# Thomi6York/pbrt-v2-skin

Measured on AMD Instinct MI355X. Metric: Msamples/s (skin.pbrt C2 pixel loop) + Mo()-gather roofline, higher is better.
Workload: dtype f32; 1 GPU; C2: skin.pbrt 1024x1024 64 spp (1024x1024, 64 spp per GPU), 128x128 tiles; scene=skin.pbrt, sampler=hash, triangles=15864, irradiance_points=2216917, tiles=64, skin_tiles=8, mo_common_grid=True

## Files before the change

### include/mpss.h

```cpp
#ifndef MPSS_H
#define MPSS_H
#include <stdint.h>

#ifdef __cplusplus
extern "C" {
#endif

#define MPSS_NBANDS 30

enum {
    MPSS_OK = 0,
    MPSS_ERR_INVALID = -1,
    MPSS_ERR_INTERNAL = -2,
    MPSS_ERR_HIP = -3,
    MPSS_ERR_NOMEM = -4
};

typedef struct mpss_ctx mpss_ctx;

typedef struct {
    int device;
    int max_depth;
    float max_error;
    float min_sample_distance;
// ... 50 lines not shown
int mpss_add_layeredskin(mpss_ctx *ctx, const mpss_layeredskin *m, uint32_t *material_id);
int mpss_update_layeredskin(mpss_ctx *ctx, uint32_t material_id, const mpss_layeredskin *m);
int mpss_build_counts(mpss_ctx *ctx, uint64_t counts[4]);
int mpss_set_material_tables(mpss_ctx *ctx, const float *rd_table, uint32_t length, const float *rcp,
                             const float *rho_hd, uint32_t n_rho, const float *albedo, int is_monte_carlo,
                             uint32_t *material_id);
int mpss_add_dipole_material(mpss_ctx *ctx, const float *sigma_a, const float *sigmap_s, float eta,
                             uint32_t *material_id);
int mpss_get_material_tables(mpss_ctx *ctx, uint32_t material_id, float *rd_table, uint32_t *length, float *rcp,
                             float *rho_hd, uint32_t *n_rho, float *total_reflectance);
int mpss_get_gather_info(mpss_ctx *ctx, uint32_t id, int *common_grid, float *rel_err, float *l1_err);

typedef struct {
    int width, height;
    const float *texels;
    int is_float;
    float shift, scale, gamma;
    int wrap;
    int trilinear;
    float max_anisotropy;
    float uscale, vscale, udelta, vdelta;
} mpss_imagemap;
void mpss_imagemap_defaults(mpss_imagemap *t);
int mpss_add_imagemap(mpss_ctx *ctx, const mpss_imagemap *t, uint32_t *texture_id);
int mpss_set_material_textures(mpss_ctx *ctx, uint32_t material_id, int32_t albedo_texture, int32_t bump_texture);

int mpss_set_irradiance_points(mpss_ctx *ctx, uint32_t n, const float *p, const float *nrm, const float *E,
                               const float *area);
int mpss_octree_info(mpss_ctx *ctx, uint32_t *n_nodes, uint32_t *max_depth, uint32_t *n_points);
int mpss_octree_export(mpss_ctx *ctx, void *nodes, float *node_et, float *pt_hdr, float *pt_e, int32_t *pt_index);

int mpss_mo_batch(mpss_ctx *ctx, uint32_t material_id, uint32_t q, const float *p_dev, float *mo_dev,
                  int32_t *counters_dev, void *stream);

int mpss_add_mesh(mpss_ctx *ctx, uint32_t nverts, const float *P, const float *N, const float *S, const float *uv,
                  uint32_t ntris, const int32_t *indices, const float *obj_to_world, const float *world_to_obj,
                  int reverse_orientation, uint32_t material_id);
int mpss_add_sphere_light(mpss_ctx *ctx, const float *center, float radius, const float *Lemit, int nsamples);
int mpss_add_infinite_light(mpss_ctx *ctx, const float *L, int nsamples, const float *light_to_world,
                            const float *world_to_light);
int mpss_add_infinite_light_map(mpss_ctx *ctx, const float *L, int nsamples, const float *light_to_world,
                                const float *world_to_light, int width, int height, const float *texels);
int mpss_set_camera(mpss_ctx *ctx, const float *raster_to_camera, const float *camera_to_world, int xres, int yres);
int mpss_set_surface_points(mpss_ctx *ctx, uint32_t n, const void *records);
int mpss_get_surface_points(mpss_ctx *ctx, void *records, uint32_t *n);
int mpss_load_pointsfile(mpss_ctx *ctx, const char *path);
int mpss_save_pointsfile(mpss_ctx *ctx, const char *path);
int mpss_get_irradiance(mpss_ctx *ctx, float *E, uint32_t *n);
int mpss_replay_samples(mpss_ctx *ctx, int spp, float *out, uint64_t *n_floats, int *k);
int mpss_preprocess(mpss_ctx *ctx, uint32_t seed);
int mpss_render_tile(mpss_ctx *ctx, int spp, uint32_t seed, int x0, int x1, int y0, int y1, float *xyzw_dev,
                     void *stream);
int mpss_render_tiles(mpss_ctx *ctx, int spp, uint32_t seed, int n, const int32_t *rects, float *const *xyzw_dev,
                      void *stream);

int mpss_tile_costs(mpss_ctx *ctx, int n, const int32_t *rects, int64_t *sss_hits, int64_t *surf_hits);

typedef struct {
    double ms_irradiance, ms_camera, ms_shade, ms_film;
    int64_t n_irradiance, n_camera, n_shade, n_film;
    int64_t samples;
    int64_t sss_samples;
    int64_t mo_nodes;
    int64_t mo_points;
    int64_t group_nodes[8], group_points[8];
    int32_t group_bands[8][4];
// ... 96 lines not shown
```

### pbrt-v2-skin_amd/csrc/context.cpp

```cpp
#include "context.h"
#include "spectral.h"

#include <cstring>

namespace mpss {

Context::Context(const mpss_config &cfg) : cfg_(cfg) {
    int ndev = 0;
    MPSS_HIP(hipGetDeviceCount(&ndev));
    if (cfg.device < 0 || cfg.device >= ndev)
        throw Error(MPSS_ERR_INVALID, "mpss_create: device ordinal " + std::to_string(cfg.device) +
                                          " out of range (" + std::to_string(ndev) + " HIP devices)");
    if (cfg.mo_near_field != 10236 && cfg.mo_near_field != 5088)
        throw Error(MPSS_ERR_INVALID, "mpss_create: mo_near_field must be 10236 or 5088");
    if (cfg.mo_common_grid != 0 && cfg.mo_common_grid != 1)
        throw Error(MPSS_ERR_INVALID, "mpss_create: mo_common_grid must be 0 or 1");
    if (cfg.mo_band_dealing != 0 && cfg.mo_band_dealing != 1)
        throw Error(MPSS_ERR_INVALID, "mpss_create: mo_band_dealing must be 0 or 1");
    max_error_ = cfg.max_error;
    min_dist_ = cfg.min_sample_distance;
    if (cfg.quick_render) {
        max_error_ *= 4.f;
        min_dist_ *= 4.f;
    }
// ... 45 lines not shown
    try {
        std::lock_guard<std::mutex> g(mu_);
        ws_free_.emplace_back(ws);
        if (ws_free_.size() > kMaxIdleWorkspaces) {
            drop = std::move(ws_free_.front());
            ws_free_.erase(ws_free_.begin());
        }
    } catch (...) {
        if (!drop) drop.reset(ws);
    }
    drop.reset();
    return e;
}

void Context::release_ws(RenderWorkspace *ws, hipStream_t stream) { MPSS_HIP(release_ws_nothrow(ws, stream)); }

void Context::quiesce_locked() {
    idle_.wait(mu_, [&] { return inflight_ == 0; });
    MPSS_HIP(hipDeviceSynchronize());
}

void Context::end_inflight() {
    std::lock_guard<std::mutex> g(mu_);
    if (--inflight_ == 0) idle_.notify_all();
}

void Context::ensure_layouts() {
    if (!have_octree_) return;
    for (const auto &m : materials_)
        if (!m->dipole) dev_octree_.ensure_layout(m->dev_profile.groups);
}

void Context::mo_batch(uint32_t mid, int q, const float *p_dev, float *out_dev, int32_t *counters_dev,
                       hipStream_t stream) {
    activate();
    RenderWorkspace *ws = nullptr;
    const BandLayout *layout = nullptr;
    const Material *m = nullptr;
    int mode;
    GatherOpts opts;
    {
        std::lock_guard<std::mutex> g(mu_);
        opts = gather_opts();
        if (!have_octree_) throw Error(MPSS_ERR_INVALID, "no irradiance points: call mpss_set_irradiance_points first");
        if (mid >= materials_.size()) throw Error(MPSS_ERR_INVALID, "unknown material id " + std::to_string(mid));
        m = materials_[mid].get();
        if (m->no_bssrdf)
            throw Error(MPSS_ERR_INVALID, "material " + std::to_string(mid) + " has no profile (genprofile false)");
        mode = cfg_.exact_mo;
        if (m->dipole) {
            mode = -1;
        } else if (m->rgb && mode != 0) {
            mode = -2;
        } else if (mode == 0) {
            layout = &dev_octree_.ensure_layout(m->dev_profile.groups);
            ws = acquire_ws();
        }
        ++inflight_;
    }
    InflightGuard guard{this, ws, stream};
    if (mode == -1) {
        launch_mo_dipole(dev_octree_, m->dev_dipole.ptr, max_error_, q, p_dev, out_dev, NB, counters_dev, stream);
        return;
    }
    if (mode == -2) {
        launch_mo_rgb(dev_octree_, m->dev_rgb.ptr, m->dev_rgb_rcp.ptr, m->rgb_rcp, m->profile.length, max_error_, q,
                      p_dev, nullptr, nullptr, nullptr, 0, out_dev, NB, counters_dev, stream);
        return;
    }
    int *perm = nullptr;
    if (ws) {
        ws->reserve(ws->perm, (size_t)(((int64_t)q + 1023) / 1024 * 1024));
        perm = ws->perm.ptr;
        if (ws->pending) MPSS_HIP(hipStreamWaitEvent(stream, ws->done, 0));
    }
    launch_mo_gather(dev_octree_, layout, m->dev_profile, max_error_, q, p_dev, out_dev, NB, counters_dev,
                     ws ? ws->work.ptr : nullptr, perm, mode, opts, stream);
    guard.release();
}

void Context::activate() const { MPSS_HIP(hipSetDevice(cfg_.device)); }

void Context::gather_info(uint32_t id, int *common_grid, float *rel_err, float *l1_err) const {
    std::lock_guard<std::mutex> g(mu_);
    if (id >= materials_.size()) throw Error(MPSS_ERR_INVALID, "unknown material id " + std::to_string(id));
    const Material &m = *materials_[id];
    const bool band = !m.dipole;
    const int lay = cfg_.mo_near_field == 10236 ? 0 : 1;
    const bool on = band && cfg_.exact_mo == 0 && cfg_.mo_common_grid != 0 &&
                    (lay == 0 ? m.dev_profile.cg.on : m.dev_profile.cg_half.on);
    *common_grid = on ? 1 : 0;
    for (int c = 0; c < NB; ++c) {
        if (rel_err) rel_err[c] = band ? m.dev_profile.cg_rel_err[lay][c] : 0.f;
        if (l1_err) l1_err[c] = band ? m.dev_profile.cg_l1_err[lay][c] : 0.f;
    }
}

void Context::material_tables(uint32_t id, float *rd, uint32_t *len, float *rcp, float *rho, uint32_t *n_rho,
                              float *total) const {
    std::lock_guard<std::mutex> g(mu_);
    if (id >= materials_.size()) throw Error(MPSS_ERR_INVALID, "unknown material id " + std::to_string(id));
    const Material &m = *materials_[id];
    *len = (uint32_t)m.profile.length;
    *n_rho = (uint32_t)m.rho.hd.size();
    if (rd) memcpy(rd, m.profile.table.data(), sizeof(float) * m.profile.table.size());
    if (rcp) memcpy(rcp, m.profile.rcp, sizeof(float) * NB);
    if (rho) memcpy(rho, m.rho.hd.data(), sizeof(float) * m.rho.hd.size());
    if (total) memcpy(total, m.profile.total_reflectance, sizeof(float) * NB);
}

void Context::common_grid(uint32_t id, int near_field, float *rows, uint32_t *n_rows, int32_t *bands, float *rg,
// ... 344 lines not shown
```

### pbrt-v2-skin_amd/csrc/context.h

```cpp
#pragma once
#include <condition_variable>
#include <memory>
#include <mutex>
#include <vector>

#include "../../include/mpss.h"
#include "common.h"
#include "dipole.h"
#include "material.h"
#include "mo_kernel.h"
#include "octree.h"
#include "pixel_filter.h"
#include "replay.h"
#include "scene.h"
#include "texture_build.h"
#include "tile_plan.h"

namespace mpss {

struct RenderScene;

struct Material {
    ProfileTables profile;
    RhoTable rho;
// ... 69 lines not shown
                     float *u0lim, float *u1lim, float *u1start, uint32_t *row0, uint32_t *ubase, float *rel_err,
                     float *l1_err, float *ua, float *hinv, int *ok) const;
    void build_counts(uint64_t counts[4]) const;
    void set_irradiance_points(int n, const float *p, const float *nrm, const float *E, const float *area);
    const DeviceOctree &octree() const;
    void export_octree(void *nodes, float *node_et, float *pt_hdr, float *pt_e, int32_t *pt_index);
    uint32_t add_imagemap(const mpss_imagemap &m);
    void set_material_textures(uint32_t material, int albedo, int bump);
    std::vector<const TexView *> host_bump_views() const;
    float max_error() const { return max_error_; }
    GatherOpts gather_opts() const {
        GatherOpts o;
        o.near_field = cfg_.mo_near_field;
        o.steal = cfg_.mo_work_stealing != 0;
        o.count_noprune = cfg_.count_traversal == 2;
        o.common_grid = cfg_.mo_common_grid != 0;
        return o;
    }
    const mpss_config &config() const { return cfg_; }

    void add_mesh(uint32_t nv, const float *P, const float *N, const float *S, const float *uv, uint32_t nt,
                  const int32_t *idx, const float *o2w, const float *w2o, bool reverse, uint32_t material);
    void add_sphere_light(const float *c, float r, const float *Lemit, int nsamples);
    void add_infinite_light(const float *L, int nsamples, const float *l2w, const float *w2l, int W = 0, int H = 0,
                            const float *texels = nullptr);
    void set_camera(const float *r2c, const float *c2w, int xres, int yres);
    void set_surface_points(uint32_t n, const SurfacePoint *pts);
    void preprocess(uint32_t seed);
    void tessellate_on_gpu();
    void find_poisson_points(uint32_t seed);
    void render_tiles(int spp, uint32_t seed, int n, const int32_t *rects, float *const *outs, hipStream_t stream);
    void replay_samples(int spp, float *out, uint64_t *n_floats, int *k);
    void check_replay_lds(int spp, const char *who) const;
    void mo_batch(uint32_t mid, int q, const float *p_dev, float *out_dev, int32_t *counters_dev, hipStream_t stream);
    void tile_costs(int n, const int32_t *rects, int64_t *sss, int64_t *surf);
    std::vector<SurfacePoint> surface_points() const {
        std::lock_guard<std::mutex> g(mu_);
        return points_;
    }
    std::vector<float> irradiance() const {
        std::lock_guard<std::mutex> g(mu_);
        return irradiance_;
    }
    std::unique_lock<std::mutex> lock_device() const {
        activate();
        return std::unique_lock<std::mutex>(mu_);
    }
    bool has_octree() const { return have_octree_; }
    mpss_render_stats render_stats();
    void reset_render_stats();
    void set_grid_builder(bool on_host) {
        std::lock_guard<std::mutex> g(mu_);
        grid_on_host_ = on_host;
    }
    void set_pixel_filter(const PixelFilter &f) {
        std::lock_guard<std::mutex> g(mu_);
        filter_ = f;
    }
    void set_instrumentation(bool timing, int counting) {
        std::lock_guard<std::mutex> g(mu_);
        cfg_.kernel_timing = timing;
        cfg_.count_traversal = counting;
    }

private:
    void activate() const;
    void upload_scene();
// ... 117 lines not shown
```

### pbrt-v2-skin_amd/csrc/mo_band.h

```cpp
#pragma once
#include <cmath>
#include <cstdlib>

#include "common.h"
#include "common_grid_types.h"
#include "octree.h"

namespace mpss {

constexpr int kHist = 13;


struct RgbK {
    float w[4];
    float x[3][4];
    float y[3][4];
};

struct BandTree {
    const NodeHdr *__restrict__ nodes;
    const float4 *__restrict__ band_et;
    const float4 *__restrict__ pt_hdr;
    const float4 *__restrict__ band_e;
    const float4 *__restrict__ band_ew;
    const float *__restrict__ table;
    BandGroups groups;
    float grcp[kGroups][4];
    float grcp_max[kGroups];
    const float *leaf_r2;
    int L, n_nodes, n_points;
    float max_error, prune_f;
    CommonGrid cg;
    CommonGrid cg_half;
    int lband[kGroups][4];
    const float *rgb_refl;
    RgbK rgb_k[kGroups];
};

struct PruneLimit {
    float rcp_min, prune_f;
};
inline PruneLimit prune_limit(int L, float rcp_min) {
    const float r = rcp_min > 0.f ? rcp_min : 0.f;
// ... 290 lines not shown
                                          int hist[kHist]) {
    CgRec r;
    const float u = d2 * c.rg;
    const uint64_t m_lds = __builtin_amdgcn_ballot_w64(u < c.u0lim);
    const uint64_t m_in = __builtin_amdgcn_ballot_w64(u < c.u1lim);
    const bool p_lds = __builtin_amdgcn_inverse_ballot_w64(m_lds);
    const bool p_row = __builtin_amdgcn_inverse_ballot_w64(m_in & ~m_lds);
    const bool p_own = __builtin_amdgcn_inverse_ballot_w64(~(m_in | m_lds));
    const int path = p_lds ? 1 : (p_row ? 0 : 2);
    const float v = __builtin_fminf(u, __builtin_fmaf(u, c.hinv, c.hc));
    uint32_t orow = 32u * ((uint32_t)v + c.rowoff);
    asm volatile("" : "+v"(orow));
    if (p_lds) cg_lds(b, c, d2, r);
    asm volatile("" : "+v"(r.p01), "+v"(r.p23)::"memory");
    if (p_own) cg_own<COUNT>(b, c, table, d2, r, hist);
    asm volatile("" ::: "memory");
    if (p_row) {
        gf4v *row = (gf4v *)((const __attribute__((address_space(1))) char *)c.tab + orow);
        r.p01 = row[0];
        r.p23 = row[1];
        if (COUNT) cg_count_rows<COUNT>((uint64_t)(uintptr_t)c.tab + orow, hist);
        const float t = __builtin_amdgcn_fractf(v);
#pragma unroll
        for (int j = 0; j < 4; ++j) r.f[j] = t;
    }
    cg_count<COUNT>(b, c, d2, path, hist);
    return r;
}

template <bool COUNT>
__device__ __forceinline__ void cg_fix(const BandLane &b, const CgLane &c, const float *table, float d2, CgRec &r,
                                       int hist[kHist]) {
    const bool bad = r.p01.x != r.p01.x;
    if (__builtin_amdgcn_ballot_w64(bad) != 0 && bad) cg_own<COUNT>(b, c, table, d2, r, hist);
}
template <bool COUNT>
__device__ __forceinline__ void cg_fix2(const BandLane &b, const CgLane &c, const float *table, float d2a,
                                        CgRec &ra, float d2b, CgRec &rb, int hist[kHist]) {
    const bool bad_a = ra.p01.x != ra.p01.x, bad_b = rb.p01.x != rb.p01.x;
    if (__builtin_amdgcn_ballot_w64(bad_a || bad_b) != 0) {
        if (bad_a) cg_own<COUNT>(b, c, table, d2a, ra, hist);
        if (bad_b) cg_own<COUNT>(b, c, table, d2b, rb, hist);
    }
}

__device__ __forceinline__ CgRec cg_fetch_near(const BandLane &b, const CgLane &c, float d2) {
    CgRec r;
    cg_lds(b, c, d2, r);
    return r;
}

template <bool RGB = false>
__device__ __forceinline__ void cg_combine(const CgRec &r, const float e[4], f2v acc[2], lds_float *rk = nullptr) {
    float rd[4];
    const RdPair v[4] = {{r.p01.x, r.p01.y}, {r.p01.z, r.p01.w}, {r.p23.x, r.p23.y}, {r.p23.z, r.p23.w}};
#pragma unroll
    for (int j = 0; j < 4; ++j) {
        const float t = r.f[j];
        float d;
        asm("v_sub_f32 %0, %1, %2" : "=v"(d) : "v"(v[j].b), "v"(v[j].a));
        asm("v_fma_f32 %0, %1, %2, %3" : "=v"(rd[j]) : "v"(t), "v"(d), "v"(v[j].a));
    }
    float o[4];
    if (RGB) from_rgb4_fused(rk, rd[0], rd[1], rd[2], o);
    const float *x = RGB ? o : rd;
#pragma unroll
    for (int h = 0; h < 2; ++h)
        acc[h] = __builtin_elementwise_fma(f2v{x[2 * h], x[2 * h + 1]}, f2v{e[2 * h], e[2 * h + 1]}, acc[h]);
}

template <bool POINT, bool COUNT, int KLDS, bool RGB = false>
__device__ __forceinline__ void band_rd_accumulate(const BandLane &b, float d2, const float e[4], float w, f2v acc[2],
                                                   int hist[kHist], lds_float *rk = nullptr) {
    float f[4];
    RdPair v[4];
    band_rd_fetch<COUNT, KLDS>(b, d2, f, v, hist);
    band_rd_combine<POINT, RGB>(f, v, e, w, acc, rk);
}

__device__ __forceinline__ bool dw_below(float a, float d, float m, float m_lo, float m_hi) {
    const uint64_t m_below = __builtin_amdgcn_ballot_w64(a < d * m_lo);
    const uint64_t m_above = __builtin_amdgcn_ballot_w64(a > d * m_hi);
    bool below = __builtin_amdgcn_inverse_ballot_w64(m_below);
    if (__builtin_amdgcn_inverse_ballot_w64(~(m_below | m_above))) below = (a / d) < m;
    return below;
}

template <bool COUNT, int KLDS, bool VROWS, bool CG = false, bool RGB = false>
__device__ __forceinline__ void mo_band_traverse(const BandTree &a, int grp, float px, float py, float pz, bool valid,
                                                 float out[4], int &k_nodes, int &k_pts, int &w_nodes, int &w_pts,
                                                 int hist[kHist], const float *lt) {
    BandLane b;
#pragma unroll
    for (int j = 0; j < 4; ++j) {
        const int c = a.lband[grp][j];
        b.rcp[j] = a.grcp[grp][j];
        b.off[j] = (uint32_t)(c >= 0 ? c : 0) * (uint32_t)a.L;
    }
    lds_float *rk = (lds_float *)lt + 4 * near_row<KLDS>() - 28;
    b.lm1 = (uint32_t)(a.L - 1);
    const uint32_t lm2 = b.lm1 - 1u;
    b.klim = (uint32_t)KLDS < lm2 ? (uint32_t)KLDS : lm2;
    b.gspan = b.lm1 - b.klim;
#pragma unroll
    for (int j = 0; j < 4; ++j) b.tb[j] = VROWS ? in_vgprs(a.table + b.off[j]) : a.table + b.off[j];
    b.lt = lt;
    b.ltl = (lds_float *)lt;
    CgLane cl;
    if (CG) {
        cl.tab = a.cg.tab;
        cl.rowoff = a.cg.row0[grp] - a.cg.ubase[grp];
        cl.rg = a.cg.rg[grp];
        cl.u0lim = a.cg.u0lim[grp];
        cl.u1lim = a.cg.u1lim[grp];
        cl.hinv = in_vgpr(a.cg.hinv[grp]);
        cl.hc = a.cg.hc[grp];
#pragma unroll
        for (int j = 0; j < 4; ++j) {
            cl.lrow[j] = a.cg.lrow[grp][j];
            cl.off[j] = b.off[j];
        }
        cl.lm1 = (uint32_t)a.L - 1u;
        cl.zoff = 4u * (uint32_t)NB * (uint32_t)a.L;
    }
    f2v acc[2] = {f2v{0.f, 0.f}, f2v{0.f, 0.f}};
    const float lds_r2_lim = !a.leaf_r2 ? 0.f : CG ? a.cg.lds_r2[grp] : (float)b.klim / (a.grcp_max[grp] * 1.00001f);
    const uint32_t lds_code = __float_as_uint(lds_r2_lim) >> 16;
    const float box_lim = a.prune_f / a.groups.rcp_min[grp];
    const cptr<float4> et_g = as_const(a.band_et + (size_t)grp * a.n_nodes);
    const cptr<float4> e_g = as_const((CG ? a.band_ew : a.band_e) + (size_t)grp * a.n_points);
    const cptr<NodeHdr> nodes = as_const(a.nodes);
    const cptr<float4> pt_hdr = as_const(a.pt_hdr);
    int resume = valid ? 0 : 0x7fffffff;
    const float m_lo = a.max_error * (1.f - 0x1p-20f), m_hi = a.max_error * (1.f + 0x1p-20f);
    int node = 0;
    while (node < a.n_nodes) {
        node = __builtin_amdgcn_readfirstlane(node);
        if (COUNT) ++w_nodes;
        const NodeHdr h = nodes[node];
        asm volatile("" ::"s"(h.px), "s"(h.py), "s"(h.pz), "s"(h.sum_area), "s"(h.bminx), "s"(h.bminy),
                     "s"(h.bminz), "s"(h.bmaxx), "s"(h.bmaxy), "s"(h.bmaxz), "s"(h.skip), "s"(h.leaf_first),
                     "s"(h.flags), "s"(h.pad), "s"(h.leaf_count), "s"(h.depth));
        const int skip = h.skip;
        bool open = false;
        if (node >= resume) {
            if (COUNT) ++k_nodes;
            const float bx = fmaxf(fmaxf(h.bminx - px, px - h.bmaxx), 0.f);
            const float by = fmaxf(fmaxf(h.bminy - py, py - h.bmaxy), 0.f);
            const float bz = fmaxf(fmaxf(h.bminz - pz, pz - h.bmaxz), 0.f);
            const float box2 = __builtin_fmaf(bz, bz, __builtin_fmaf(by, by, bx * bx));
            if (box2 >= box_lim || (h.flags & NODE_BLACK)) {
                resume = skip;
            } else {
                const float dx = px - h.px, dy = py - h.py, dz = pz - h.pz;
                const float d2 = dx * dx + dy * dy + dz * dz;
                const bool inside = fmaxf(fmaxf(bx, by), bz) == 0.f;
                if (dw_below(h.sum_area, d2, a.max_error, m_lo, m_hi) && !inside) {
                    resume = skip;
                    if (CG) {
                        CgRec r = cg_fetch<COUNT>(b, cl, a.table, d2, hist);
                        int nd = node;
                        asm volatile("" : "+s"(nd)::"memory");
                        const float4 et = et_g[nd];
                        const float e[4] = {et.x, et.y, et.z, et.w};
                        cg_fix<COUNT>(b, cl, a.table, d2, r, hist);
                        cg_combine<RGB>(r, e, acc, rk);
                    } else {
                        const float4 et = et_g[node];
                        const float e[4] = {et.x, et.y, et.z, et.w};
                        band_rd_accumulate<false, COUNT, KLDS, RGB>(b, d2, e, 1.f, acc, hist, rk);
                    }
                } else {
                    open = true;
                }
            }
        }
        const bool any_open = __builtin_amdgcn_ballot_w64(open) != 0;
        if (h.leaf_first >= 0) {
            if (any_open) {
                f2v lacc[2] = {f2v{0.f, 0.f}, f2v{0.f, 0.f}};
                const int live = (int)(h.pad & 0xffffu);
                if (COUNT) w_pts += live;
                int i0 = 0;
                if (!COUNT && KLDS > 0 && (h.pad >> 16) < lds_code) {
                    for (; i0 + 1 < live; i0 += 2) {
                        const int ka = h.leaf_first + i0, kb = ka + 1;
                        const float4 pa = pt_hdr[ka], pb = pt_hdr[kb];
                        const float4 ea = e_g[ka], eb = e_g[kb];
                        if (!open) continue;
                        const float ax = px - pa.x, ay = py - pa.y, az = pz - pa.z;
                        const float bx2 = px - pb.x, by2 = py - pb.y, bz2 = pz - pb.z;
                        const float d2a = ax * ax + ay * ay + az * az;
                        const float d2b = bx2 * bx2 + by2 * by2 + bz2 * bz2;
                        const float e0[4] = {ea.x, ea.y, ea.z, ea.w}, e1[4] = {eb.x, eb.y, eb.z, eb.w};
                        if (CG) {
                            const CgRec ra = cg_fetch_near(b, cl, d2a), rb = cg_fetch_near(b, cl, d2b);
                            cg_combine<RGB>(ra, e0, lacc, rk);
                            cg_combine<RGB>(rb, e1, lacc, rk);
                            continue;
                        }
                        float fa[4], fb[4];
                        RdPair va[4], vb[4];
                        band_rd_fetch_lds<KLDS>(b, d2a, fa, va);
                        band_rd_fetch_lds<KLDS>(b, d2b, fb, vb);
                        band_rd_combine<true, RGB>(fa, va, e0, pa.w, lacc, rk);
                        band_rd_combine<true, RGB>(fb, vb, e1, pb.w, lacc, rk);
                    }
                }
                for (; i0 + 1 < live; i0 += 2) {
                        const int ka = h.leaf_first + i0, kb = ka + 1;
                        const float4 pa = pt_hdr[ka], pb = pt_hdr[kb];
                        const float4 ea = e_g[ka], eb = e_g[kb];
                        if (!COUNT)
                            asm volatile("" ::"s"(pa.x), "s"(pa.y), "s"(pa.z), "s"(pa.w), "s"(pb.x), "s"(pb.y),
                                         "s"(pb.z), "s"(pb.w), "s"(ea.x), "s"(ea.y), "s"(ea.z), "s"(ea.w),
// ... 20 lines not shown
                        if (!COUNT)
                            asm volatile("" ::"v"(va[0].a), "v"(va[0].b), "v"(va[1].a), "v"(va[1].b), "v"(va[2].a),
                                         "v"(va[2].b), "v"(va[3].a), "v"(va[3].b), "v"(vb[0].a), "v"(vb[0].b),
                                         "v"(vb[1].a), "v"(vb[1].b), "v"(vb[2].a), "v"(vb[2].b), "v"(vb[3].a),
                                         "v"(vb[3].b));
                        const float e0[4] = {ea.x, ea.y, ea.z, ea.w}, e1[4] = {eb.x, eb.y, eb.z, eb.w};
                        band_rd_combine<true, RGB>(fa, va, e0, pa.w, lacc, rk);
                        band_rd_combine<true, RGB>(fb, vb, e1, pb.w, lacc, rk);
                    }
                for (int i = i0; i < live; ++i) {
                    const int kp = h.leaf_first + i;
                    const float4 ph = pt_hdr[kp];
                    if (!open) continue;
                    if (COUNT) ++k_pts;
                    const float ex = px - ph.x, ey = py - ph.y, ez = pz - ph.z;
                    const float d2 = ex * ex + ey * ey + ez * ez;
                    if (CG) {
                        CgRec r = cg_fetch<COUNT>(b, cl, a.table, d2, hist);
                        int kq = kp;
                        asm volatile("" : "+s"(kq)::"memory");
                        const float4 ev = e_g[kq];
                        const float e[4] = {ev.x, ev.y, ev.z, ev.w};
                        cg_fix<COUNT>(b, cl, a.table, d2, r, hist);
                        cg_combine<RGB>(r, e, lacc, rk);
                    } else {
                        const float4 ev = e_g[kp];
                        const float e[4] = {ev.x, ev.y, ev.z, ev.w};
                        band_rd_accumulate<true, COUNT, KLDS, RGB>(b, d2, e, ph.w, lacc, hist, rk);
                    }
                }
                acc[0] += lacc[0];
                acc[1] += lacc[1];
            }
            if (open) resume = skip;
            node = skip;
        } else if (any_open) {
            node = node + 1;
        } else {
            node = skip;
        }
    }
    out[0] = acc[0].x;
    out[1] = acc[0].y;
    out[2] = acc[1].x;
    out[3] = acc[1].y;
}
#endif

}
```

### pbrt-v2-skin_amd/csrc/mo_kernel.h

```cpp
#pragma once
#include "common.h"
#include "device_octree.h"
#include "mo_band.h"

namespace mpss {

struct DeviceProfile {
    DevBuf<float> table;
    DevBuf<float> rcp;
    float rcp_min = 0.f;
    int L = 0;
    float host_rcp[NB];
    BandGroups groups{};
    DevBuf<float4> ctab, ctab_half;
    CommonGrid cg{}, cg_half{};
    float cg_rel_err[2][NB] = {};
    float cg_l1_err[2][NB] = {};
    void upload(const float *table, int L, const float *rcp, bool snake = false, bool grid_host = true);
    bool grid_on_host = true;
    void build_common(const float *table, const BandGroups &slots, int lds_reserve, bool rgb);
    DevBuf<float> rgb_refl;
    void set_rgb(const float *table);
};

struct GatherOpts {
    int near_field = 10236;
    bool steal = true;
    bool count_noprune = false;
    bool common_grid = true;
};

void launch_mo_gather(const DeviceOctree &t, const BandLayout *layout, const DeviceProfile &p, float max_error, int nq,
                      const float *queries, float *out, int out_stride, int32_t *counters, int *work, int *perm,
                      int mode, const GatherOpts &opts, hipStream_t stream);

void launch_mo_exact(const DeviceOctree &t, const DeviceProfile &p, float max_error, int nq, const float *queries,
                     float *out, int out_stride, int32_t *counters, hipStream_t stream);
void launch_mo_packet(const DeviceOctree &t, const DeviceProfile &p, float max_error, int nq, const float *queries,
                      float *out, int out_stride, int32_t *counters, hipStream_t stream);

void launch_mo_dipole(const DeviceOctree &t, const float *dipole_dev, float max_error, int nq, const float *queries,
                      float *out, int out_stride, int32_t *counters, hipStream_t stream);

void launch_mo_rgb(const DeviceOctree &t, const float *table3, const float *rcp3_dev, const float rcp3[3], int L,
                   float max_error, int nq, const float *queries, const float4 *queries4, const int *count_dev,
                   const uint32_t *hit_s, int mat, float *out, int out_stride, int32_t *counters, hipStream_t stream);

constexpr int kStatStride = 4 + 13;

void launch_mo_band(const DeviceOctree &t, const BandLayout &layout, const DeviceProfile &p, float max_error,
                    int nq_max, const float4 *queries4, const int *count_dev, float4 *out4,
                    const uint32_t *hit_s, int mat, unsigned long long *counts, int *work, int *perm,
                    const GatherOpts &opts, hipStream_t stream);

}
```

### pbrt-v2-skin_amd/csrc/mo_kernel.hip

```cpp
#include "mo_kernel.h"
#include "mo_wave.h"
#include "spectral.h"

#include <algorithm>
#include <cmath>

namespace mpss {

namespace {

__device__ __forceinline__ uint32_t morton_expand10(uint32_t v) {
    v &= 0x3ffu;
    v = (v | (v << 16)) & 0x030000ffu;
    v = (v | (v << 8)) & 0x0300f00fu;
    v = (v | (v << 4)) & 0x030c30c3u;
    v = (v | (v << 2)) & 0x09249249u;
    return v;
}
__device__ __forceinline__ uint32_t morton30(float x, float y, float z, const float lo[3], const float inv[3]) {
    const float q[3] = {(x - lo[0]) * inv[0], (y - lo[1]) * inv[1], (z - lo[2]) * inv[2]};
    uint32_t c[3];
#pragma unroll
    for (int k = 0; k < 3; ++k) c[k] = (uint32_t)fminf(fmaxf(q[k], 0.f), 1023.f);
    return (morton_expand10(c[0]) << 2) | (morton_expand10(c[1]) << 1) | morton_expand10(c[2]);
// ... 112 lines not shown
    bt.n_nodes = t.n_nodes;
    bt.n_points = t.n_points;
    bt.max_error = max_error;
    const PruneLimit pl = prune_limit(p.L, p.rcp_min);
    bt.prune_f = pl.prune_f;
    if (!(pl.rcp_min > 0.f))
        for (int g = 0; g < kGroups; ++g) bt.groups.rcp_min[g] = 0.f;
    return bt;
}

}

void launch_mo_band(const DeviceOctree &t, const BandLayout &layout, const DeviceProfile &p, float max_error,
                    int nq_max, const float4 *queries4, const int *count_dev, float4 *out4, const uint32_t *hit_s,
                    int mat, unsigned long long *counts, int *work, int *perm, const GatherOpts &opts,
                    hipStream_t stream) {
    if (nq_max <= 0 || t.n_nodes <= 0) return;
    BandArgs a{};
    a.t = band_tree(t, layout, p, max_error);
    a.queries4 = queries4;
    a.count = count_dev;
    a.hit_s = hit_s;
    a.mat = mat;
    a.nq = nq_max;
    a.out4 = out4;
    a.counts = counts;
    a.work = work;
    a.perm = perm;
    launch_band(a, nq_max, t, counts != nullptr, opts, stream);
}

void launch_mo_gather(const DeviceOctree &t, const BandLayout *layout, const DeviceProfile &p, float max_error, int nq,
                      const float *queries, float *out, int out_stride, int32_t *counters, int *work, int *perm,
                      int mode, const GatherOpts &opts, hipStream_t stream) {
    if (nq <= 0) return;
    if (t.n_nodes <= 0) throw Error(-1, "launch_mo_gather: octree is empty");
    if (p.L < 2) throw Error(-1, "launch_mo_gather: profile table has fewer than 2 entries");
    if (mode == 1) return launch_mo_exact(t, p, max_error, nq, queries, out, out_stride, counters, stream);
    if (mode != 0) return launch_mo_packet(t, p, max_error, nq, queries, out, out_stride, counters, stream);
    const bool count = counters != nullptr;
    if (!layout || !work) throw Error(-2, "launch_mo_gather: the sharded gather needs a band layout and work counters");
    if (count) MPSS_HIP(hipMemsetAsync(counters, 0, sizeof(int32_t) * 4 * (size_t)nq, stream));
    BandArgs b{};
    b.t = band_tree(t, *layout, p, max_error);
    b.queries3 = queries;
    b.nq = nq;
    b.out = out;
    b.out_stride = out_stride;
    b.counters = counters;
    b.work = work;
    b.perm = perm;
    launch_band(b, nq, t, count, opts, stream);
}

}
```

### pbrt-v2-skin_amd/csrc/mo_wave.h

```cpp
#pragma once
#include "mo_kernel.h"
#include "mo_band.h"

namespace mpss {


struct BandArgs {
    BandTree t;
    const float *__restrict__ queries3;
    const float4 *__restrict__ queries4;
    const int *__restrict__ count;
    const uint32_t *__restrict__ hit_s;
    int mat;
    int nq;
    float *__restrict__ out;
    float4 *__restrict__ out4;
    int out_stride;
    int32_t *__restrict__ counters;
    unsigned long long *__restrict__ counts;
    int *__restrict__ work;
    float klo[3], kinv[3];
    int *perm;
    int steal;
};

__device__ __forceinline__ bool band_query(const BandArgs &a, int q, float &px, float &py, float &pz) {
    if (a.queries4) {
        const float4 v = a.queries4[q];
        px = v.x;
        py = v.y;
        pz = v.z;
        bool live = v.w >= 0.f;
        if (live && a.hit_s) live = (int)((a.hit_s[q] >> 16) & 0xffu) == a.mat;
        return live;
    }
    px = a.queries3[3 * (size_t)q];
    py = a.queries3[3 * (size_t)q + 1];
// ... 126 lines not shown
```

### pbrt-v2-skin_amd/csrc/mpss_abi.cpp

```cpp
#include <algorithm>
#include <cmath>
#include <cstring>
#include <memory>
#include <string>
#include <vector>

#include "../../include/mpss.h"
#include "common_grid.h"
#include "context.h"
#include "material.h"
#include "mc_profile.h"
#include "mo_kernel.h"
#include "profile_fit.h"
#include "profile_fit_driver.h"
#include "sog_fit.h"
#include "spectral.h"

using namespace mpss;

namespace {
thread_local std::string g_last_error;

template <class F>
int guarded(F &&fn) {
// ... 256 lines not shown
        require(c && p && nrm && E && area, "mpss_set_irradiance_points: null argument");
        require(n > 0, "mpss_set_irradiance_points: empty point set");
        require(n <= (1u << 30), "mpss_set_irradiance_points: at most 2^30 points");
        reinterpret_cast<Context *>(c)->set_irradiance_points((int)n, p, nrm, E, area);
    });
}

int mpss_octree_info(mpss_ctx *c, uint32_t *nn, uint32_t *md, uint32_t *np) {
    return guarded([&] {
        require(c, "mpss_octree_info: null ctx");
        const DeviceOctree &t = reinterpret_cast<Context *>(c)->octree();
        if (nn) *nn = (uint32_t)t.n_nodes;
        if (md) *md = (uint32_t)t.max_depth;
        if (np) *np = (uint32_t)t.n_points;
    });
}

int mpss_octree_export(mpss_ctx *c, void *nodes, float *node_et, float *pt_hdr, float *pt_e, int32_t *pt_index) {
    return guarded([&] {
        require(c, "mpss_octree_export: null ctx");
        reinterpret_cast<Context *>(c)->export_octree(nodes, node_et, pt_hdr, pt_e, pt_index);
    });
}

int mpss_mo_batch(mpss_ctx *c, uint32_t id, uint32_t q, const float *p_dev, float *mo_dev, int32_t *counters_dev,
                  void *stream) {
    return guarded([&] {
        require(c && (q == 0 || (p_dev && mo_dev)), "mpss_mo_batch: null argument");
        require(q <= (1u << 30), "mpss_mo_batch: at most 2^30 queries per call");
        reinterpret_cast<Context *>(c)->mo_batch(id, (int)q, p_dev, mo_dev, counters_dev, (hipStream_t)stream);
    });
}

int mpss_add_mesh(mpss_ctx *c, uint32_t nv, const float *P, const float *N, const float *S, const float *uv,
                  uint32_t nt, const int32_t *idx, const float *o2w, const float *w2o, int rev, uint32_t mat) {
    return guarded([&] {
        require(c && P && idx && o2w && w2o && nv > 0 && nt > 0, "mpss_add_mesh: bad argument");
        reinterpret_cast<Context *>(c)->add_mesh(nv, P, N, S, uv, nt, idx, o2w, w2o, rev != 0, mat);
    });
}

int mpss_add_sphere_light(mpss_ctx *c, const float *center, float r, const float *L, int ns) {
    return guarded([&] {
        require(c && center && L, "mpss_add_sphere_light: null argument");
        reinterpret_cast<Context *>(c)->add_sphere_light(center, r, L, ns);
    });
}

int mpss_add_infinite_light(mpss_ctx *c, const float *L, int ns, const float *l2w, const float *w2l) {
    return guarded([&] {
        require(c && L && l2w && w2l, "mpss_add_infinite_light: null argument");
        reinterpret_cast<Context *>(c)->add_infinite_light(L, ns, l2w, w2l);
    });
}

int mpss_add_infinite_light_map(mpss_ctx *c, const float *L, int ns, const float *l2w, const float *w2l, int w, int h,
                                const float *texels) {
    return guarded([&] {
        require(c && L && l2w && w2l && texels, "mpss_add_infinite_light_map: null argument");
        reinterpret_cast<Context *>(c)->add_infinite_light(L, ns, l2w, w2l, w, h, texels);
    });
}

int mpss_set_camera(mpss_ctx *c, const float *r2c, const float *c2w, int xres, int yres) {
    return guarded([&] {
        require(c && r2c && c2w, "mpss_set_camera: null argument");
// ... 444 lines not shown
```

### pbrt-v2-skin_amd/mpss/__init__.py

```python
import ctypes as C
import os

import numpy as np

NB = 30
_HERE = os.path.dirname(os.path.abspath(__file__))
LIB_PATH = os.environ.get("MPSS_LIB") or os.path.join(_HERE, "libmpss.so")

if not os.path.exists(LIB_PATH):
    raise ImportError("libmpss.so not built (%s): run __graft_entry__.build() or make -C pbrt-v2-skin_amd/csrc"
                      % LIB_PATH)

try:
    import torch
except ImportError:
    torch = None

_lib = C.CDLL(LIB_PATH)

f32p = np.ctypeslib.ndpointer(dtype=np.float32, flags="C_CONTIGUOUS")
i32p = np.ctypeslib.ndpointer(dtype=np.int32, flags="C_CONTIGUOUS")
vp = C.c_void_p
u32 = C.c_uint32
u32p = C.POINTER(C.c_uint32)
# ... 50 lines not shown
                ("n_f_blood", C.c_uint32), ("n_f_ohg", C.c_uint32), ("layer_thickness_nm", C.c_float * 2),
                ("layer_ior", C.c_float * 2), ("desired_length", C.c_int), ("id_min", C.c_int), ("id_max", C.c_int),
                ("max_profiles_per_batch", C.c_int)]


def _sig(name, res, args):
    f = getattr(_lib, name)
    f.restype = res
    f.argtypes = args
    return f


_sig("mpss_abi_version", C.c_int, [])
_sig("mpss_last_error", C.c_char_p, [])
_sig("mpss_config_defaults", None, [C.POINTER(Config)])
_sig("mpss_create", C.c_int, [C.POINTER(Config), C.POINTER(vp)])
_sig("mpss_destroy", None, [vp])
_sig("mpss_layeredskin_defaults", None, [C.POINTER(LayeredSkin)])
_sig("mpss_add_layeredskin", C.c_int, [vp, C.POINTER(LayeredSkin), u32p])
_sig("mpss_update_layeredskin", C.c_int, [vp, u32, C.POINTER(LayeredSkin)])
_sig("mpss_build_counts", C.c_int, [vp, C.POINTER(C.c_uint64)])
_sig("mpss_get_common_grid", C.c_int, [vp, u32, C.c_int, vp, u32p] + [vp] * 11 + [C.POINTER(C.c_int)])
_sig("mpss_set_grid_builder", C.c_int, [vp, C.c_int])
_sig("mpss_set_pixel_filter", C.c_int, [vp, C.c_int, C.c_float, C.c_float, C.c_float, C.c_float])
_sig("mpss_set_material_tables", C.c_int, [vp, f32p, u32, f32p, f32p, u32, vp, C.c_int, u32p])
_sig("mpss_add_dipole_material", C.c_int, [vp, f32p, f32p, C.c_float, u32p])
_sig("mpss_host_dipole_rd", C.c_int, [f32p, f32p, C.c_float, u32, vp, vp, vp])
_sig("mpss_get_material_tables", C.c_int, [vp, u32, vp, u32p, vp, vp, u32p, vp])
_sig("mpss_get_gather_info", C.c_int, [vp, u32, C.POINTER(C.c_int), vp, vp])
_sig("mpss_set_irradiance_points", C.c_int, [vp, u32, f32p, f32p, f32p, f32p])
_sig("mpss_octree_info", C.c_int, [vp, u32p, u32p, u32p])
_sig("mpss_octree_export", C.c_int, [vp, vp, vp, vp, vp, vp])
_sig("mpss_mo_batch", C.c_int, [vp, u32, u32, vp, vp, vp, vp])
_sig("mpss_add_mesh", C.c_int, [vp, u32, f32p, vp, vp, vp, u32, C.POINTER(C.c_int32), f32p, f32p, C.c_int, u32])
_sig("mpss_add_sphere_light", C.c_int, [vp, f32p, C.c_float, f32p, C.c_int])
_sig("mpss_add_infinite_light", C.c_int, [vp, f32p, C.c_int, f32p, f32p])
_sig("mpss_add_infinite_light_map", C.c_int, [vp, f32p, C.c_int, f32p, f32p, C.c_int, C.c_int, f32p])
_sig("mpss_set_camera", C.c_int, [vp, f32p, f32p, C.c_int, C.c_int])
_sig("mpss_set_surface_points", C.c_int, [vp, u32, vp])
_sig("mpss_get_surface_points", C.c_int, [vp, vp, u32p])
_sig("mpss_get_irradiance", C.c_int, [vp, vp, u32p])
_sig("mpss_replay_samples", C.c_int, [vp, C.c_int, vp, C.POINTER(C.c_uint64), C.POINTER(C.c_int)])
_sig("mpss_load_pointsfile", C.c_int, [vp, C.c_char_p])
_sig("mpss_save_pointsfile", C.c_int, [vp, C.c_char_p])
_sig("mpss_preprocess", C.c_int, [vp, u32])
_sig("mpss_get_render_stats", C.c_int, [vp, C.POINTER(RenderStats)])
_sig("mpss_reset_render_stats", C.c_int, [vp])
_sig("mpss_set_instrumentation", C.c_int, [vp, C.c_int, C.c_int])
_sig("mpss_render_tile", C.c_int, [vp, C.c_int, u32, C.c_int, C.c_int, C.c_int, C.c_int, vp, vp])
_sig("mpss_render_tiles", C.c_int, [vp, C.c_int, u32, C.c_int, C.POINTER(C.c_int32), C.POINTER(vp), vp])
_sig("mpss_tile_costs", C.c_int, [vp, C.c_int, C.POINTER(C.c_int32), vp, vp])
_sig("mpss_host_from_rgb", C.c_int, [f32p, C.c_int, f32p])
_sig("mpss_mc_reference", C.c_int, [f32p, C.c_int, C.c_float, C.c_int, C.c_int, vp, vp, C.POINTER(C.c_double),
                                    C.POINTER(C.c_double)])
_sig("mpss_mc_profile", C.c_int, [vp, f32p, C.c_int, C.c_float, C.c_int, C.c_uint64, C.c_uint64, vp, vp,
                                  C.POINTER(C.c_double), C.POINTER(C.c_double), C.POINTER(C.c_uint64), vp])
_sig("mpss_mc_profile_batch", C.c_int, [vp, vp, C.c_int, C.c_int, C.c_float, C.c_int, C.c_uint64, C.c_uint64, vp, vp,
                                        vp, vp, C.POINTER(C.c_uint64), vp])
_sig("mpss_mc_reference_batch", C.c_int, [vp, vp, C.c_int, C.c_int, C.c_float, C.c_int, C.c_int, C.c_int, C.c_int,
                                          vp, vp, vp, vp, vp])
_sig("mpss_host_tessellate", C.c_int, [u32, f32p, vp, vp, vp, u32, C.POINTER(C.c_int32), f32p, f32p, C.c_int, u32,
                                       C.c_float, C.c_int, vp, u32p])
_sig("mpss_imagemap_defaults", None, [C.POINTER(Imagemap)])
_sig("mpss_add_imagemap", C.c_int, [vp, C.POINTER(Imagemap), u32p])
_sig("mpss_set_material_textures", C.c_int, [vp, u32, C.c_int32, C.c_int32])
_sig("mpss_host_tessellate_bumped", C.c_int, [u32, f32p, vp, vp, vp, u32, C.POINTER(C.c_int32), f32p, f32p, C.c_int,
# ... 427 lines not shown
        rcp = np.zeros(NB, np.float32)
        rho = np.zeros(nr.value, np.float32)
        tot = np.zeros(NB, np.float32)
        check(_lib.mpss_get_material_tables(self.h, mid, tab.ctypes.data, C.byref(L), rcp.ctypes.data,
                                            rho.ctypes.data, C.byref(nr), tot.ctypes.data))
        return tab, rcp, rho, tot

    def gather_info(self, mid):
        on = C.c_int()
        rel = np.zeros(NB, np.float32)
        l1 = np.zeros(NB, np.float32)
        check(_lib.mpss_get_gather_info(self.h, mid, C.byref(on), rel.ctypes.data, l1.ctypes.data))
        return dict(common_grid=bool(on.value), rel_err=rel, l1_err=l1)

    def set_irradiance_points(self, p, n, E, area):
        p, n, E, area = [np.ascontiguousarray(x, np.float32) for x in (p, n, E, area)]
        check(_lib.mpss_set_irradiance_points(self.h, len(p), p, n, E, area))

    def octree_info(self):
        a, b, c = C.c_uint32(), C.c_uint32(), C.c_uint32()
        check(_lib.mpss_octree_info(self.h, C.byref(a), C.byref(b), C.byref(c)))
        return dict(n_nodes=a.value, max_depth=b.value, n_points=c.value)

    def octree_export(self):
        info = self.octree_info()
        N, M = info["n_nodes"], info["n_points"]
        d = dict(nodes=np.zeros((N, 16), np.uint32), node_et=np.zeros((N, 32), np.float32),
                 pt_hdr=np.zeros((M, 4), np.float32), pt_e=np.zeros((M, 32), np.float32),
                 pt_index=np.zeros(M, np.int32))
        check(_lib.mpss_octree_export(self.h, *[d[k].ctypes.data_as(vp) for k in
                                                ("nodes", "node_et", "pt_hdr", "pt_e", "pt_index")]))
        return d

    def mo_batch(self, mid, q, p_dev, mo_dev, counters_dev=None, stream=None):
        check(_lib.mpss_mo_batch(self.h, mid, q, p_dev, mo_dev, counters_dev, stream))

    def add_mesh(self, P, idx, o2w, w2o, material, N=None, S=None, uv=None, reverse=False):
        P = np.ascontiguousarray(P, np.float32).reshape(-1, 3)
        idx = np.ascontiguousarray(idx, np.int32).reshape(-1, 3)
        opt = [None if a is None else np.ascontiguousarray(a, np.float32) for a in (N, S, uv)]
        self._keep = opt
        check(_lib.mpss_add_mesh(self.h, len(P), P, *[None if a is None else a.ctypes.data for a in opt],
                                 len(idx), idx.ctypes.data_as(C.POINTER(C.c_int32)),
                                 np.ascontiguousarray(o2w, np.float32), np.ascontiguousarray(w2o, np.float32),
                                 int(reverse), material))

    def add_imagemap(self, **tex):
        t, keep = imagemap(**tex)
        tid = C.c_uint32(0)
        check(_lib.mpss_add_imagemap(self.h, C.byref(t), C.byref(tid)))
        del keep
        return tid.value

    def set_material_textures(self, material, albedo=-1, bump=-1):
        check(_lib.mpss_set_material_textures(self.h, material, albedo, bump))

    def add_sphere_light(self, center, radius, Lemit, nsamples=1):
        check(_lib.mpss_add_sphere_light(self.h, np.ascontiguousarray(center, np.float32), radius,
                                         np.ascontiguousarray(Lemit, np.float32), nsamples))

    def add_infinite_light(self, L, nsamples=1, light_to_world=None, world_to_light=None, texels=None):
        l2w = np.eye(4, dtype=np.float32) if light_to_world is None else light_to_world
        w2l = np.linalg.inv(np.asarray(l2w, np.float64)) if world_to_light is None else world_to_light
        args = (self.h, np.ascontiguousarray(L, np.float32), nsamples, np.ascontiguousarray(l2w, np.float32),
                np.ascontiguousarray(w2l, np.float32))
        if texels is None:
# ... 134 lines not shown
```

Measured before the change: 1489 Msamples/s.

## Compute octree walk decisions as wave masks and add gather path statistics

The octree walk in the band gather now evaluates the node test for every lane unconditionally and keeps active, near, accepted and open lanes as 64-bit ballot masks. The tie case in the distance-weighted test only runs when some lane needs it, and the resume update is taken from the masks instead of per-lane branches. A new API entry, mpss_mo_batch_paths, returns per-group counts of which walk paths were taken, and the histogram grows from 13 to 19 slots. The aim is less branch divergence and fewer redundant ballots in the hot walk, in exchange for extra box and distance arithmetic on lanes that would otherwise sit idle.

```diff
diff --git a/include/mpss.h b/include/mpss.h
--- a/include/mpss.h
+++ b/include/mpss.h
@@ -106,6 +106,11 @@
 
 int mpss_mo_batch(mpss_ctx *ctx, uint32_t material_id, uint32_t q, const float *p_dev, float *mo_dev,
                   int32_t *counters_dev, void *stream);
+
+#define MPSS_MO_PATH_GROUPS 8
+#define MPSS_MO_PATH_STATS 23
+int mpss_mo_batch_paths(mpss_ctx *ctx, uint32_t material_id, uint32_t q, const float *p_dev, float *mo_dev,
+                        uint64_t *stats);
 
 int mpss_add_mesh(mpss_ctx *ctx, uint32_t nverts, const float *P, const float *N, const float *S, const float *uv,
                   uint32_t ntris, const int32_t *indices, const float *obj_to_world, const float *world_to_obj,
diff --git a/pbrt-v2-skin_amd/csrc/context.cpp b/pbrt-v2-skin_amd/csrc/context.cpp
--- a/pbrt-v2-skin_amd/csrc/context.cpp
+++ b/pbrt-v2-skin_amd/csrc/context.cpp
@@ -101,7 +101,7 @@
 }
 
 void Context::mo_batch(uint32_t mid, int q, const float *p_dev, float *out_dev, int32_t *counters_dev,
-                       hipStream_t stream) {
+                       hipStream_t stream, unsigned long long *counts_dev) {
     activate();
     RenderWorkspace *ws = nullptr;
     const BandLayout *layout = nullptr;
@@ -128,6 +128,8 @@
         ++inflight_;
     }
     InflightGuard guard{this, ws, stream};
+    if (counts_dev && mode != 0)
+        throw Error(MPSS_ERR_INVALID, "path statistics come from the sharded gather only (exact_mo 0, a tabulated profile)");
     if (mode == -1) {
         launch_mo_dipole(dev_octree_, m->dev_dipole.ptr, max_error_, q, p_dev, out_dev, NB, counters_dev, stream);
         return;
@@ -144,8 +146,20 @@
         if (ws->pending) MPSS_HIP(hipStreamWaitEvent(stream, ws->done, 0));
     }
     launch_mo_gather(dev_octree_, layout, m->dev_profile, max_error_, q, p_dev, out_dev, NB, counters_dev,
-                     ws ? ws->work.ptr : nullptr, perm, mode, opts, stream);
+                     ws ? ws->work.ptr : nullptr, perm, mode, opts, stream, counts_dev);
     guard.release();
+}
+
+void Context::mo_batch_paths(uint32_t mid, int q, const float *p_dev, float *out_dev, uint64_t *stats) {
+    activate();
+    const size_t n = (size_t)kStatStride * kGroups;
+    DevBuf<unsigned long long> d;
+    d.alloc(n);
+    MPSS_HIP(hipMemset(d.ptr, 0, n * sizeof(unsigned long long)));
+    mo_batch(mid, q, p_dev, out_dev, nullptr, nullptr, d.ptr);
+    MPSS_HIP(hipStreamSynchronize(nullptr));
+    static_assert(sizeof(unsigned long long) == sizeof(uint64_t), "the statistics are 64-bit counts");
+    MPSS_HIP(hipMemcpy(stats, d.ptr, n * sizeof(uint64_t), hipMemcpyDeviceToHost));
 }
 
 void Context::activate() const { MPSS_HIP(hipSetDevice(cfg_.device)); }
diff --git a/pbrt-v2-skin_amd/csrc/context.h b/pbrt-v2-skin_amd/csrc/context.h
--- a/pbrt-v2-skin_amd/csrc/context.h
+++ b/pbrt-v2-skin_amd/csrc/context.h
@@ -125,7 +125,9 @@
     void render_tiles(int spp, uint32_t seed, int n, const int32_t *rects, float *const *outs, hipStream_t stream);
     void replay_samples(int spp, float *out, uint64_t *n_floats, int *k);
     void check_replay_lds(int spp, const char *who) const;
-    void mo_batch(uint32_t mid, int q, const float *p_dev, float *out_dev, int32_t *counters_dev, hipStream_t stream);
+    void mo_batch(uint32_t mid, int q, const float *p_dev, float *out_dev, int32_t *counters_dev, hipStream_t stream,
+                  unsigned long long *counts_dev = nullptr);
+    void mo_batch_paths(uint32_t mid, int q, const float *p_dev, float *out_dev, uint64_t *stats);
     void tile_costs(int n, const int32_t *rects, int64_t *sss, int64_t *surf);
     std::vector<SurfacePoint> surface_points() const {
         std::lock_guard<std::mutex> g(mu_);
diff --git a/pbrt-v2-skin_amd/csrc/mo_band.h b/pbrt-v2-skin_amd/csrc/mo_band.h
--- a/pbrt-v2-skin_amd/csrc/mo_band.h
+++ b/pbrt-v2-skin_amd/csrc/mo_band.h
@@ -8,7 +8,7 @@
 
 namespace mpss {
 
-constexpr int kHist = 13;
+constexpr int kHist = 19;
 
 
 struct RgbK {
@@ -365,12 +365,14 @@
 __device__ __forceinline__ void cg_fix(const BandLane &b, const CgLane &c, const float *table, float d2, CgRec &r,
                                        int hist[kHist]) {
     const bool bad = r.p01.x != r.p01.x;
+    if (COUNT && bad) ++hist[13];
     if (__builtin_amdgcn_ballot_w64(bad) != 0 && bad) cg_own<COUNT>(b, c, table, d2, r, hist);
 }
 template <bool COUNT>
 __device__ __forceinline__ void cg_fix2(const BandLane &b, const CgLane &c, const float *table, float d2a,
                                         CgRec &ra, float d2b, CgRec &rb, int hist[kHist]) {
     const bool bad_a = ra.p01.x != ra.p01.x, bad_b = rb.p01.x != rb.p01.x;
+    if (COUNT) hist[13] += (int)bad_a + (int)bad_b;
     if (__builtin_amdgcn_ballot_w64(bad_a || bad_b) != 0) {
         if (bad_a) cg_own<COUNT>(b, c, table, d2a, ra, hist);
         if (bad_b) cg_own<COUNT>(b, c, table, d2b, rb, hist);
@@ -411,11 +413,11 @@
     band_rd_combine<POINT, RGB>(f, v, e, w, acc, rk);
 }
 
-__device__ __forceinline__ bool dw_below(float a, float d, float m, float m_lo, float m_hi) {
-    const uint64_t m_below = __builtin_amdgcn_ballot_w64(a < d * m_lo);
-    const uint64_t m_above = __builtin_amdgcn_ballot_w64(a > d * m_hi);
-    bool below = __builtin_amdgcn_inverse_ballot_w64(m_below);
-    if (__builtin_amdgcn_inverse_ballot_w64(~(m_below | m_above))) below = (a / d) < m;
+__device__ __forceinline__ uint64_t dw_below(float a, float d, float m, float m_lo, float m_hi, uint64_t lanes) {
+    uint64_t below = __builtin_amdgcn_ballot_w64(a < d * m_lo);
+    const uint64_t above = __builtin_amdgcn_ballot_w64(a > d * m_hi);
+    const uint64_t tie = lanes & ~(below | above);
+    if (tie != 0) below |= tie & __builtin_amdgcn_ballot_w64((a / d) < m);
     return below;
 }
 
@@ -475,45 +477,57 @@
                      "s"(h.bminz), "s"(h.bmaxx), "s"(h.bmaxy), "s"(h.bmaxz), "s"(h.skip), "s"(h.leaf_first),
                      "s"(h.flags), "s"(h.pad), "s"(h.leaf_count), "s"(h.depth));
         const int skip = h.skip;
-        bool open = false;
-        if (node >= resume) {
-            if (COUNT) ++k_nodes;
-            const float bx = fmaxf(fmaxf(h.bminx - px, px - h.bmaxx), 0.f);
-            const float by = fmaxf(fmaxf(h.bminy - py, py - h.bmaxy), 0.f);
-            const float bz = fmaxf(fmaxf(h.bminz - pz, pz - h.bmaxz), 0.f);
-            const float box2 = __builtin_fmaf(bz, bz, __builtin_fmaf(by, by, bx * bx));
-            if (box2 >= box_lim || (h.flags & NODE_BLACK)) {
-                resume = skip;
-            } else {
-                const float dx = px - h.px, dy = py - h.py, dz = pz - h.pz;
-                const float d2 = dx * dx + dy * dy + dz * dz;
-                const bool inside = fmaxf(fmaxf(bx, by), bz) == 0.f;
-                if (dw_below(h.sum_area, d2, a.max_error, m_lo, m_hi) && !inside) {
-                    resume = skip;
-                    if (CG) {
-                        CgRec r = cg_fetch<COUNT>(b, cl, a.table, d2, hist);
-                        int nd = node;
-                        asm volatile("" : "+s"(nd)::"memory");
-                        const float4 et = et_g[nd];
-                        const float e[4] = {et.x, et.y, et.z, et.w};
-                        cg_fix<COUNT>(b, cl, a.table, d2, r, hist);
-                        cg_combine<RGB>(r, e, acc, rk);
-                    } else {
-                        const float4 et = et_g[node];
-                        const float e[4] = {et.x, et.y, et.z, et.w};
-                        band_rd_accumulate<false, COUNT, KLDS, RGB>(b, d2, e, 1.f, acc, hist, rk);
-                    }
+        const uint64_t m_act = __builtin_amdgcn_ballot_w64(node >= resume);
+        if (COUNT && __builtin_amdgcn_inverse_ballot_w64(m_act)) ++k_nodes;
+        const float bx = fmaxf(fmaxf(h.bminx - px, px - h.bmaxx), 0.f);
+        const float by = fmaxf(fmaxf(h.bminy - py, py - h.bmaxy), 0.f);
+        const float bz = fmaxf(fmaxf(h.bminz - pz, pz - h.bmaxz), 0.f);
+        const float box2 = __builtin_fmaf(bz, bz, __builtin_fmaf(by, by, bx * bx));
+        const uint64_t m_near =
+            (h.flags & NODE_BLACK) ? 0 : m_act & __builtin_amdgcn_ballot_w64(!(box2 >= box_lim));
+        if (COUNT && __builtin_amdgcn_inverse_ballot_w64(m_act)) {
+            if (h.flags & NODE_BLACK)
+                ++hist[17];
+            else if (box2 >= box_lim)
+                ++hist[16];
+        }
+        uint64_t m_open = 0;
+        if (m_near != 0) {
+            const float dx = px - h.px, dy = py - h.py, dz = pz - h.pz;
+            const float d2 = dx * dx + dy * dy + dz * dz;
+            const uint64_t m_out = __builtin_amdgcn_ballot_w64(fmaxf(fmaxf(bx, by), bz) != 0.f);
+            if (COUNT && node > 0 && __builtin_amdgcn_inverse_ballot_w64(m_near & ~m_out)) ++hist[18];
+            const uint64_t m_acc = m_near & m_out & dw_below(h.sum_area, d2, a.max_error, m_lo, m_hi, m_near);
+            m_open = m_near & ~m_acc;
+            if (__builtin_amdgcn_inverse_ballot_w64(m_acc)) {
+                if (CG) {
+                    CgRec r = cg_fetch<COUNT>(b, cl, a.table, d2, hist);
+                    int nd = node;
+                    asm volatile("" : "+s"(nd)::"memory");
+                    const float4 et = et_g[nd];
+                    const float e[4] = {et.x, et.y, et.z, et.w};
+                    cg_fix<COUNT>(b, cl, a.table, d2, r, hist);
+                    cg_combine<RGB>(r, e, acc, rk);
                 } else {
-                    open = true;
+                    const float4 et = et_g[node];
+                    const float e[4] = {et.x, et.y, et.z, et.w};
+                    band_rd_accumulate<false, COUNT, KLDS, RGB>(b, d2, e, 1.f, acc, hist, rk);
                 }
             }
         }
-        const bool any_open = __builtin_amdgcn_ballot_w64(open) != 0;
+        const bool open = __builtin_amdgcn_inverse_ballot_w64(m_open);
+        const bool any_open = m_open != 0;
+        const uint64_t m_closed = h.leaf_first >= 0 ? m_act : m_act & ~m_open;
+        if (__builtin_amdgcn_inverse_ballot_w64(m_closed)) resume = skip;
         if (h.leaf_first >= 0) {
             if (any_open) {
                 f2v lacc[2] = {f2v{0.f, 0.f}, f2v{0.f, 0.f}};
                 const int live = (int)(h.pad & 0xffffu);
                 if (COUNT) w_pts += live;
+                if (COUNT && open) {
+                    hist[14] += KLDS > 0 && (h.pad >> 16) < lds_code && live > 1;
+                    hist[15] += live & 1;
+                }
                 int i0 = 0;
                 if (!COUNT && KLDS > 0 && (h.pad >> 16) < lds_code) {
                     for (; i0 + 1 < live; i0 += 2) {
@@ -600,7 +614,6 @@
                 acc[0] += lacc[0];
                 acc[1] += lacc[1];
             }
-            if (open) resume = skip;
             node = skip;
         } else if (any_open) {
             node = node + 1;
diff --git a/pbrt-v2-skin_amd/csrc/mo_kernel.h b/pbrt-v2-skin_amd/csrc/mo_kernel.h
--- a/pbrt-v2-skin_amd/csrc/mo_kernel.h
+++ b/pbrt-v2-skin_amd/csrc/mo_kernel.h
@@ -32,7 +32,7 @@
 
 void launch_mo_gather(const DeviceOctree &t, const BandLayout *layout, const DeviceProfile &p, float max_error, int nq,
                       const float *queries, float *out, int out_stride, int32_t *counters, int *work, int *perm,
-                      int mode, const GatherOpts &opts, hipStream_t stream);
+                      int mode, const GatherOpts &opts, hipStream_t stream, unsigned long long *counts = nullptr);
 
 void launch_mo_exact(const DeviceOctree &t, const DeviceProfile &p, float max_error, int nq, const float *queries,
                      float *out, int out_stride, int32_t *counters, hipStream_t stream);
@@ -46,7 +46,7 @@
                    float max_error, int nq, const float *queries, const float4 *queries4, const int *count_dev,
                    const uint32_t *hit_s, int mat, float *out, int out_stride, int32_t *counters, hipStream_t stream);
 
-constexpr int kStatStride = 4 + 13;
+constexpr int kStatStride = 4 + 19;
 
 void launch_mo_band(const DeviceOctree &t, const BandLayout &layout, const DeviceProfile &p, float max_error,
                     int nq_max, const float4 *queries4, const int *count_dev, float4 *out4,
diff --git a/pbrt-v2-skin_amd/csrc/mo_kernel.hip b/pbrt-v2-skin_amd/csrc/mo_kernel.hip
--- a/pbrt-v2-skin_amd/csrc/mo_kernel.hip
+++ b/pbrt-v2-skin_amd/csrc/mo_kernel.hip
@@ -168,15 +168,16 @@
 
 void launch_mo_gather(const DeviceOctree &t, const BandLayout *layout, const DeviceProfile &p, float max_error, int nq,
                       const float *queries, float *out, int out_stride, int32_t *counters, int *work, int *perm,
-                      int mode, const GatherOpts &opts, hipStream_t stream) {
+                      int mode, const GatherOpts &opts, hipStream_t stream, unsigned long long *counts) {
     if (nq <= 0) return;
+    if (counts && mode != 0) throw Error(-1, "launch_mo_gather: path statistics come from the sharded gather only");
     if (t.n_nodes <= 0) throw Error(-1, "launch_mo_gather: octree is empty");
     if (p.L < 2) throw Error(-1, "launch_mo_gather: profile table has fewer than 2 entries");
     if (mode == 1) return launch_mo_exact(t, p, max_error, nq, queries, out, out_stride, counters, stream);
     if (mode != 0) return launch_mo_packet(t, p, max_error, nq, queries, out, out_stride, counters, stream);
-    const bool count = counters != nullptr;
+    const bool count = counters != nullptr || counts != nullptr;
     if (!layout || !work) throw Error(-2, "launch_mo_gather: the sharded gather needs a band layout and work counters");
-    if (count) MPSS_HIP(hipMemsetAsync(counters, 0, sizeof(int32_t) * 4 * (size_t)nq, stream));
+    if (counters) MPSS_HIP(hipMemsetAsync(counters, 0, sizeof(int32_t) * 4 * (size_t)nq, stream));
     BandArgs b{};
     b.t = band_tree(t, *layout, p, max_error);
     b.queries3 = queries;
@@ -184,6 +185,7 @@
     b.out = out;
     b.out_stride = out_stride;
     b.counters = counters;
+    b.counts = counts;
     b.work = work;
     b.perm = perm;
     launch_band(b, nq, t, count, opts, stream);
diff --git a/pbrt-v2-skin_amd/csrc/mo_wave.h b/pbrt-v2-skin_amd/csrc/mo_wave.h
--- a/pbrt-v2-skin_amd/csrc/mo_wave.h
+++ b/pbrt-v2-skin_amd/csrc/mo_wave.h
@@ -3,6 +3,8 @@
 #include "mo_band.h"
 
 namespace mpss {
+
+static_assert(kStatStride == 4 + kHist, "the statistics hold the walk's four counts and every kHist slot");
 
 
 struct BandArgs {
diff --git a/pbrt-v2-skin_amd/csrc/mpss_abi.cpp b/pbrt-v2-skin_amd/csrc/mpss_abi.cpp
--- a/pbrt-v2-skin_amd/csrc/mpss_abi.cpp
+++ b/pbrt-v2-skin_amd/csrc/mpss_abi.cpp
@@ -312,6 +312,14 @@
     });
 }
 
+int mpss_mo_batch_paths(mpss_ctx *c, uint32_t id, uint32_t q, const float *p_dev, float *mo_dev, uint64_t *stats) {
+    return guarded([&] {
+        require(c && p_dev && mo_dev && stats && q > 0, "mpss_mo_batch_paths: null argument");
+        require(q <= (1u << 30), "mpss_mo_batch_paths: at most 2^30 queries per call");
+        reinterpret_cast<Context *>(c)->mo_batch_paths(id, (int)q, p_dev, mo_dev, stats);
+    });
+}
+
 int mpss_add_mesh(mpss_ctx *c, uint32_t nv, const float *P, const float *N, const float *S, const float *uv,
                   uint32_t nt, const int32_t *idx, const float *o2w, const float *w2o, int rev, uint32_t mat) {
     return guarded([&] {
diff --git a/pbrt-v2-skin_amd/mpss/__init__.py b/pbrt-v2-skin_amd/mpss/__init__.py
--- a/pbrt-v2-skin_amd/mpss/__init__.py
+++ b/pbrt-v2-skin_amd/mpss/__init__.py
@@ -106,6 +106,7 @@
 _sig("mpss_octree_info", C.c_int, [vp, u32p, u32p, u32p])
 _sig("mpss_octree_export", C.c_int, [vp, vp, vp, vp, vp, vp])
 _sig("mpss_mo_batch", C.c_int, [vp, u32, u32, vp, vp, vp, vp])
+_sig("mpss_mo_batch_paths", C.c_int, [vp, u32, u32, vp, vp, vp])
 _sig("mpss_add_mesh", C.c_int, [vp, u32, f32p, vp, vp, vp, u32, C.POINTER(C.c_int32), f32p, f32p, C.c_int, u32])
 _sig("mpss_add_sphere_light", C.c_int, [vp, f32p, C.c_float, f32p, C.c_int])
 _sig("mpss_add_infinite_light", C.c_int, [vp, f32p, C.c_int, f32p, f32p])
@@ -599,6 +600,11 @@
                                                 ("nodes", "node_et", "pt_hdr", "pt_e", "pt_index")]))
         return d
 
+    def mo_batch_paths(self, mid, q, p_dev, mo_dev):
+        stats = np.zeros((8, 23), np.uint64)
+        check(_lib.mpss_mo_batch_paths(self.h, mid, q, p_dev, mo_dev, stats.ctypes.data))
+        return stats
+
     def mo_batch(self, mid, q, p_dev, mo_dev, counters_dev=None, stream=None):
         check(_lib.mpss_mo_batch(self.h, mid, q, p_dev, mo_dev, counters_dev, stream))
 
```

Result: faster. 1508 Msamples/s, median of 6 (+1.3%).
